# lbarseghyan/diffusion-models

Measured on AMD Instinct MI355X. Metric: sampled images/sec, 32x32 U-Net (dim 64, mults 1-2-4-8), DDPM-1000, higher is better.
Workload: dtype f32; 1 GPU; ddpm1000_32x32_unet64_b256_per_gpu; sampler=p_sample_loop (DDPM), sampler_steps=1000, batch_per_gpu=256, global_batch=256, hip_graph=True, graph_captures=1, parallelism=batch-shard x1, one all-gather per sample()

## Files before the change

### diffusion-models_amd/_lib.py

```python
from __future__ import annotations

import ctypes as C
import os
from typing import Optional

import torch

_HERE = os.path.dirname(os.path.abspath(__file__))
LIB_PATH = os.environ.get("DM_LIB") or os.path.join(_HERE, "libdm_hip.so")
DM_MAX_STAGES = 8
DM_COEFS = 8
DM_EDM_COEFS = 16
EDM_HEUN, EDM_DPMPP = 0, 1
DM_CT_COEFS = 16
CT_PRED_NOISE, CT_PRED_V = 0, 1
DM_REPAINT_COEFS = 16
DM_LV_COEFS = 16
DM_LV_TRAIN_COEFS = 12
DM_WO_COEFS = 16
DM_WO_TRAIN_COEFS = 12
DM_CG_COEFS = 16
ABI_VERSION = 9
DDIM_NO_CLAMP, DDIM_RAW_NOISE = 1, 2

# ... 19 lines not shown
    "dm_op_mse_loss", "dm_op_adam_step", "dm_op_ema_lerp",
    "dm_unet_optimizer_step", "dm_unet_train_scalar", "dm_unet_ema_update", "dm_unet_get_param", "dm_unet_set_train_tensor", "dm_unet_adam_step",
    "dm_unet_train_sync", "dm_unet_check_device_pack",
    "dm_unet_train_dropout", "dm_op_dropout_mask",
    "dm_op_conv2d_bwd", "dm_op_downsample_bwd", "dm_op_block_bwd", "dm_op_rmsnorm_bwd", "dm_op_linear_attention_bwd",
    "dm_op_attention_bwd", "dm_op_cross_attention", "dm_op_cross_attention_bwd",
    "dm_op_linear_attention_core_bwd", "dm_op_attention_core_bwd",
    "dm_profile_enable", "dm_profile_read",
    "dm_unet_forward_ft", "dm_sample_edm",
    "dm_op_edm_churn_in", "dm_op_edm_euler", "dm_op_edm_heun", "dm_op_edm_dpmpp", "dm_op_edm_finalize",
    "dm_unet_train_enable_ft", "dm_unet_loss_backward_edm",
    "dm_op_edm_noise_in", "dm_op_edm_loss", "dm_op_sinusoid_ft_bwd",
    "dm_sample_ct", "dm_unet_loss_backward_ct", "dm_op_ct_step", "dm_op_ct_noise_in", "dm_op_ct_loss",
    "dm_unet_loss_backward_ct_ig", "dm_op_conv7_dgrad", "dm_op_sinusoid_ft_tgrad", "dm_op_ct_sched_reduce",
    "dm_sample_ct_dpmpp", "dm_op_ct_dpmpp_step",
    "dm_unet_optimizer_step_ex",
    "dm_sample_repaint", "dm_op_repaint_step",
    "dm_sample_lv", "dm_unet_loss_backward_lv", "dm_op_lv_step", "dm_op_lv_loss",
    "dm_sample_wo", "dm_unet_loss_backward_wo", "dm_op_wo_step", "dm_op_wo_loss",
    "dm_sample_classifier_guided", "dm_op_cg_mean", "dm_op_cg_finish",
    "dm_op_dpmpp_update",
    "dm_sample_ex_dyn", "dm_op_dyn_threshold", "dm_op_sampler_update_dyn", "dm_op_dpmpp_update_dyn",
    "dm_unet_cond_forward", "dm_unet_cond_backward", "dm_op_deferred_reduce",
)


class UnetCfg(C.Structure):
    _fields_ = [
        ("dim", C.c_int32), ("init_dim", C.c_int32), ("out_dim", C.c_int32), ("channels", C.c_int32),
        ("input_channels", C.c_int32), ("n_stages", C.c_int32),
        ("dim_mults", C.c_int32 * DM_MAX_STAGES), ("full_attn", C.c_int32 * DM_MAX_STAGES),
        ("attn_heads", C.c_int32), ("attn_dim_head", C.c_int32),
        ("text_mode", C.c_int32), ("text_emb_dim", C.c_int32), ("sinusoidal_theta", C.c_float),
        ("learned_sinusoidal_dim", C.c_int32), ("attn_heads_stage", C.c_int32 * DM_MAX_STAGES),
        ("seq1d", C.c_int32),
    ]


class DecoderCfg(C.Structure):
    _fields_ = [
        ("ch", C.c_int32), ("out_ch", C.c_int32), ("n_levels", C.c_int32), ("ch_mult", C.c_int32 * DM_MAX_STAGES),
        ("num_res_blocks", C.c_int32), ("n_attn_res", C.c_int32), ("attn_resolutions", C.c_int32 * DM_MAX_STAGES),
        ("resolution", C.c_int32), ("z_channels", C.c_int32), ("embed_dim", C.c_int32),
    ]


# ... 193 lines not shown
    lib.dm_decoder_create.argtypes = [C.POINTER(DecoderCfg), i32, C.POINTER(vp)]
    lib.dm_decoder_destroy.argtypes = [vp]
    lib.dm_decoder_destroy.restype = None
    lib.dm_decoder_set_param.argtypes = [vp, C.c_char_p, fp, C.POINTER(i64), i32]
    lib.dm_decoder_missing_params.argtypes = [vp]
    lib.dm_decoder_finalize.argtypes = [vp]
    lib.dm_decoder_forward.argtypes = [vp, fp, fp, i32, i32, i32, vp]
    lib.dm_encoder_create.argtypes = [C.POINTER(EncoderCfg), i32, C.POINTER(vp)]
    lib.dm_encoder_destroy.argtypes = [vp]
    lib.dm_encoder_destroy.restype = None
    lib.dm_encoder_set_param.argtypes = [vp, C.c_char_p, fp, C.POINTER(i64), i32]
    lib.dm_encoder_missing_params.argtypes = [vp]
    lib.dm_encoder_finalize.argtypes = [vp]
    lib.dm_encoder_forward.argtypes = [vp, fp, fp, fp, vp, i32, i32, i32, vp]
    lib.dm_encoder_forward_kl.argtypes = [vp, fp, fp, fp, fp, fp, u64, u64, u64, i32, i32, i32, i32, vp]
    lib.dm_encoder_quantize.argtypes = [vp, fp, fp, vp, i32, i32, i32, vp]
    lib.dm_encoder_embed_code.argtypes = [vp, vp, fp, i32, i32, i32, vp]
    lib.dm_op_conv2d.argtypes = [fp, i32, fp, i32, fp, fp, fp, fp, i32, i32, i32, i32, i32, i32, i32, vp]
    lib.dm_op_downsample.argtypes = [fp, i32, fp, fp, fp, i32, i32, i32, i32, vp]
    lib.dm_op_rmsnorm.argtypes = [fp, fp, fp, i32, i32, i32, i32, vp]
    lib.dm_op_block.argtypes = [fp, i32, fp, fp, fp, fp, fp, fp, i32, i32, i32, i32, vp]
    lib.dm_op_linear_attention.argtypes = [fp, fp, fp, fp, fp, fp, fp, fp, i32, i32, i32, i32, i32, i32, vp]
    lib.dm_op_attention.argtypes = [fp, fp, fp, fp, fp, fp, fp, i32, i32, i32, i32, i32, i32, vp]
    lib.dm_op_sampler_update.argtypes = [i32, i32, fp, fp, fp, C.POINTER(C.c_float), fp, fp, i64, vp]
    lib.dm_op_sampler_update_ex.argtypes = [i32, i32, i32, fp, fp, fp, C.POINTER(C.c_float), fp, fp, i64, vp]
    lib.dm_op_conv1d.argtypes = [fp, i32, fp, i32, fp, fp, fp, fp, i32, i32, i32, i32, i32, i32, i32, vp]
    lib.dm_op_block1d.argtypes = [fp, i32, fp, i32, fp, fp, fp, fp, fp, fp, fp, i32, i32, i32, vp]
    lib.dm_op_dpmpp_update.argtypes = [i32, fp, fp, fp, C.POINTER(C.c_float), fp, i64, vp]
    lib.dm_op_dyn_threshold.argtypes = [i32, fp, fp, C.POINTER(C.c_float), i32, i64, C.c_double, fp, vp]
    lib.dm_op_sampler_update_dyn.argtypes = [i32, i32, fp, fp, fp, C.POINTER(C.c_float), fp, i32, i64, fp, fp, vp]
    lib.dm_op_dpmpp_update_dyn.argtypes = [i32, fp, fp, fp, C.POINTER(C.c_float), fp, i32, i64, fp, vp]
    lib.dm_op_cfg_combine.argtypes = [fp, fp, fp, i32, i64, C.c_float, C.c_float, i32, C.c_float, vp]
    lib.dm_op_group_norm.argtypes = [fp, fp, fp, fp, i32, i32, i32, i32, C.c_float, i32, vp]
    lib.dm_op_vae_attention.argtypes = [fp, fp, fp, fp, i32, i32, i32, i32, vp]
    lib.dm_op_vq_nearest.argtypes = [fp, fp, fp, vp, i64, i32, i32, i32, vp]
    lib.dm_op_vq_nearest_nchw.argtypes = [fp, fp, fp, vp, i64, i32, i32, i32, vp]
    lib.dm_op_kl_posterior.argtypes = [fp, i32, fp, u64, u64, u64, i32, fp, fp, fp, i32, i32, i32, vp]
    lib.dm_op_embed_code.argtypes = [vp, i32, fp, fp, i64, i32, i32, i32, vp]
    lib.dm_conv_create.argtypes = [fp, fp, i32, i32, i32, i32, i32, i32, i32, i32, i32, C.POINTER(vp)]
    lib.dm_conv_destroy.argtypes = [vp]
    lib.dm_conv_destroy.restype = None
    lib.dm_conv_forward.argtypes = [vp, fp, i32, i32, i32, i32, fp, vp]
    lib.dm_op_pool2d.argtypes = [fp, fp, i32, i32, i32, i32, i32, i32, i32, i32, vp]
    lib.dm_op_resize_bilinear.argtypes = [fp, fp, i32, i32, i32, i32, i32, i32, fp, fp, vp]
    lib.dm_op_copy_channels_nhwc.argtypes = [fp, i32, fp, i32, i32, i64, vp]
    lib.dm_op_global_avgpool.argtypes = [fp, fp, i32, i32, i32, vp]
# ... 161 lines not shown
```

### diffusion-models_amd/csrc/attn16_fused.hip

```cpp
#include "conv_device.h"

#include <cmath>
#include <cstdlib>
#include <vector>

namespace dm {

static constexpr int A16_OS = 132;
static constexpr int A16_D = 4;

bool attn16_eligible(int dim, int heads, int dh) {
    static const bool off = env_flag("DM_NO_ATTN16");
    return !off && heads == 4 && dh == 32 && dim % 256 == 0 && dim >= 256 && dim <= 1024;
}

void attn16_pack(const float* w_qkv, const float* norm_g, const float* w_out, int C, std::vector<float>& wp,
                 std::vector<float>& wo) {
    const float sc = std::sqrt((float)C), qs = 1.0f / std::sqrt(32.0f);
    wp.assign((size_t)384 * C, 0.f);
    for (int s = 0; s < C / 16; ++s)
        for (int t = 0; t < 24; ++t)
            for (int lane = 0; lane < 64; ++lane)
                for (int j = 0; j < 4; ++j) {
                    const int row = 16 * t + (lane & 15), ch = 16 * s + 4 * (lane >> 4) + j;
                    float v = w_qkv[(size_t)row * C + ch] * norm_g[ch] * sc;
                    if (row < 128) v *= qs;
                    wp[(((size_t)s * 24 + t) * 64 + lane) * 4 + j] = v;
                }
    wo.assign((size_t)C * 128, 0.f);
    for (int s = 0; s < 8; ++s)
        for (int ct = 0; ct < C / 16; ++ct)
            for (int lane = 0; lane < 64; ++lane)
                for (int j = 0; j < 4; ++j)
                    wo[(((size_t)s * (C / 16) + ct) * 64 + lane) * 4 + j] =
                        w_out[(size_t)(16 * ct + (lane & 15)) * 128 + 16 * s + 4 * (lane >> 4) + j];
}

__device__ __forceinline__ f32x4 a16_mfma(float a, float b, f32x4 c) {
    return __builtin_amdgcn_mfma_f32_16x16x4f32(a, b, c, 0, 0, 0);
}

__global__ __launch_bounds__(256) void attn16_fused_kernel(const float* __restrict__ x, const Attn16 w,
                                                            float* __restrict__ y, int add_x) {
    extern __shared__ __attribute__((aligned(16))) float smem[];
    const int C = w.C;
    const int XS = C + 4;
    float* xs = smem;
    float* ol = smem + 16 * XS;
    const int tid = threadIdx.x;
    const int lane = tid & 63;
    const int h = __builtin_amdgcn_readfirstlane(tid >> 6);
    const int l15 = lane & 15, kq = lane >> 4;
    const size_t img = blockIdx.x;

    const int S = C / 16;
    const float* wl = w.wp + (size_t)lane * 4;
    f32x4 wr[A16_D][6];
    auto load = [&](int s, int d) {
        const float* ws = wl + (size_t)s * (24 * 256);
#pragma unroll
        for (int part = 0; part < 3; ++part)
#pragma unroll
            for (int t = 0; t < 2; ++t)
                wr[d][2 * part + t] = *reinterpret_cast<const f32x4*>(ws + (8 * part + 2 * h + t) * 256);
    };
#pragma unroll
    for (int d = 0; d < A16_D; ++d) load(min(d, S - 1), d);

    {
        const int token = tid >> 4, li = tid & 15;
        const float* xr = x + (img * 16 + token) * C;
        f32x4 xv[16];
        float ss = 0.f;
#pragma unroll
        for (int i = 0; i < 16; ++i) {
            const int c = 4 * li + 64 * i;
            if (c < C) {
                xv[i] = *reinterpret_cast<const f32x4*>(xr + c);
                ss += xv[i].x * xv[i].x + xv[i].y * xv[i].y + xv[i].z * xv[i].z + xv[i].w * xv[i].w;
            }
        }
        ss += dpp_f<0xB1>(ss);
        ss += dpp_f<0x4E>(ss);
        ss += dpp_f<0x141>(ss);
        ss += dpp_f<0x140>(ss);
        const float rn = fast_rsq(fmaxf(ss, 1e-24f));
#pragma unroll
        for (int i = 0; i < 16; ++i) {
            const int c = 4 * li + 64 * i;
            if (c < C) *reinterpret_cast<f32x4*>(xs + token * XS + c) = xv[i] * rn;
        }
    }
    __syncthreads();

    const f32x4 z4 = make_f32x4(0.f, 0.f, 0.f, 0.f);
    f32x4 qT[2] = {z4, z4}, kT[2] = {z4, z4}, vv[2] = {z4, z4};
    {
        const float* xrow = xs + l15 * XS + 4 * kq;
        for (int s = 0; s < S; s += A16_D) {
#pragma unroll
            for (int d = 0; d < A16_D; ++d) {
                if (s + d < S) {
                    const f32x4 xa = *reinterpret_cast<const f32x4*>(xrow + 16 * (s + d));
#pragma unroll
                    for (int j = 0; j < 4; ++j) {
#pragma unroll
                        for (int t = 0; t < 2; ++t) {
                            qT[t] = a16_mfma(wr[d][t][j], xa[j], qT[t]);
                            kT[t] = a16_mfma(wr[d][2 + t][j], xa[j], kT[t]);
                            vv[t] = a16_mfma(xa[j], wr[d][4 + t][j], vv[t]);
                        }
                    }
                    if (s + d + A16_D < S) load(s + d + A16_D, d);
                }
            }
        }
    }

    const int CT = C / 16;
    const int ct_per_wave = CT / 4;
    const int n_it = (ct_per_wave / 4) * 8;
    const float* wol = w.wo + (size_t)lane * 4;
    f32x4 wv4[4][4];
    auto load_o = [&](int it, int slot) {
        const int c0 = (it >> 3) * 4, so = it & 7;
#pragma unroll
        for (int i = 0; i < 4; ++i)
            wv4[slot][i] = *reinterpret_cast<const f32x4*>(wol + ((size_t)so * CT + h * ct_per_wave + c0 + i) * 256);
    };
#pragma unroll
    for (int d = 0; d < 4; ++d) load_o(d, d);

    const float* mk = w.mem_kv + (size_t)h * 4 * 32;
    const float* mv = w.mem_kv + (size_t)(4 + h) * 4 * 32;
    f32x4 st = z4, sm = z4;
#pragma unroll
    for (int t = 0; t < 2; ++t) {
        const f32x4 km = l15 < 4 ? *reinterpret_cast<const f32x4*>(mk + l15 * 32 + 16 * t + 4 * kq) : z4;
#pragma unroll
        for (int e = 0; e < 4; ++e) {
            st = a16_mfma(kT[t][e], qT[t][e], st);
            sm = a16_mfma(km[e], qT[t][e], sm);
        }
    }
    const bool g0 = kq == 0;
    float mx = fmaxf(fmaxf(st.x, st.y), fmaxf(st.z, st.w));
    if (g0) mx = fmaxf(mx, fmaxf(fmaxf(sm.x, sm.y), fmaxf(sm.z, sm.w)));
    mx = fmaxf(mx, __shfl_xor(mx, 16));
    mx = fmaxf(mx, __shfl_xor(mx, 32));
    f32x4 pt, pm;
    pt.x = __expf(st.x - mx);
    pt.y = __expf(st.y - mx);
    pt.z = __expf(st.z - mx);
    pt.w = __expf(st.w - mx);
    pm.x = g0 ? __expf(sm.x - mx) : 0.f;
    pm.y = g0 ? __expf(sm.y - mx) : 0.f;
    pm.z = g0 ? __expf(sm.z - mx) : 0.f;
    pm.w = g0 ? __expf(sm.w - mx) : 0.f;
    float sum = (pt.x + pt.y) + (pt.z + pt.w) + (pm.x + pm.y) + (pm.z + pm.w);
    sum += __shfl_xor(sum, 16);
    sum += __shfl_xor(sum, 32);
    const float inv = 1.0f / sum;
    pt = pt * inv;
    pm = pm * inv;

#pragma unroll
    for (int t = 0; t < 2; ++t) {
        f32x4 ot = z4;
        f32x4 vm = z4;
        if (g0) {
            vm.x = mv[0 * 32 + 16 * t + l15];
            vm.y = mv[1 * 32 + 16 * t + l15];
            vm.z = mv[2 * 32 + 16 * t + l15];
            vm.w = mv[3 * 32 + 16 * t + l15];
        }
#pragma unroll
        for (int e = 0; e < 4; ++e) {
            ot = a16_mfma(vv[t][e], pt[e], ot);
            ot = a16_mfma(vm[e], pm[e], ot);
        }
        *reinterpret_cast<f32x4*>(ol + l15 * A16_OS + h * 32 + 16 * t + 4 * kq) = ot;
    }
    __syncthreads();

    f32x4 ob[8];
#pragma unroll
    for (int s = 0; s < 8; ++s) ob[s] = *reinterpret_cast<const f32x4*>(ol + l15 * A16_OS + 16 * s + 4 * kq);
    const size_t row = (img * 16 + l15) * C;
    for (int c0 = 0; c0 < ct_per_wave; c0 += 4) {
        f32x4 acc[4] = {z4, z4, z4, z4};
        const int it0 = (c0 >> 2) * 8;
#pragma unroll
        for (int s = 0; s < 8; ++s) {
#pragma unroll
            for (int j = 0; j < 4; ++j)
#pragma unroll
                for (int i = 0; i < 4; ++i) acc[i] = a16_mfma(wv4[s & 3][i][j], ob[s][j], acc[i]);
            if (it0 + s + 4 < n_it) load_o(it0 + s + 4, s & 3);
        }
#pragma unroll
        for (int i = 0; i < 4; ++i) {
            const int c = 16 * (h * ct_per_wave + c0 + i) + 4 * kq;
            f32x4 r = acc[i] + *reinterpret_cast<const f32x4*>(w.bias + c);
            if (add_x) r += *reinterpret_cast<const f32x4*>(x + row + c);
            *reinterpret_cast<f32x4*>(y + row + c) = r;
        }
    }
}

int launch_attn16_fused(const Attn16& w, const float* x, float* y, int B, bool add_x, hipStream_t s) {
    DM_REQUIRE(w.C % 256 == 0 && w.C >= 256 && w.C <= 1024 && B > 0, "attn16: channel count");
    const size_t lds = (size_t)(16 * (w.C + 4) + 16 * A16_OS) * sizeof(float);
    static LdsOptIn lds_flag;
    if (lds_opt_in(lds_flag, reinterpret_cast<const void*>(attn16_fused_kernel), 1)) return 1;
    const bool timed = prof::enabled();
    if (timed) {
        const double tok = 16.0 * B;
        const double flops = 2.0 * tok * (384.0 * w.C + 128.0 * w.C + 2.0 * 4 * 20 * 32);
        const double bytes = 4.0 * (2.0 * tok * w.C + 512.0 * w.C);
        if (prof::begin("attn16_fused_kernel", flops, bytes, s)) return 1;
    }
    hipLaunchKernelGGL(attn16_fused_kernel, dim3(B), dim3(256), lds, s, x, w, y, add_x ? 1 : 0);
    DM_CHECK_HIP(hipGetLastError());
    if (timed && prof::end(s)) return 1;
    return 0;
}

}
```

### diffusion-models_amd/csrc/dm_api.hip

```cpp
#include "../../include/dm_hip.h"
#include "dm_common.h"
#include "edm.h"
#include "ct.h"
#include "repaint.h"
#include "learned.h"
#include "weighted.h"
#include "cguide.h"

#include <array>
#include <cmath>
#include <cstdlib>
#include <cstring>
#include <functional>
#include <map>
#include <memory>
#include <set>
#include <stdexcept>
#include <string>
#include <unordered_map>
#include <vector>

namespace dm {

static thread_local std::string g_err;
// ... 615 lines not shown
        ob += mb.data.size();
    }
    return 0;
}

static int fuse_linattn(DeviceOwner& own, AttnLayer& A, const float* w_qkv, const float* norm_g, const float* w_out,
                        const float* mem_kv, const float* out_g, int dim, int heads, int dh) {
    A.has_fused = false;
    if (!linattn_fused_eligible(dim, heads, dh)) return 0;
    std::vector<float> wq, wk, wv, wo, kb;
    if (!linattn_fused_pack(w_qkv, norm_g, w_out, mem_kv, dim, wq, wk, wv, wo, kb)) return 0;
    std::vector<float> ogs(out_g, out_g + dim);
    for (float& v : ogs) v *= std::sqrt((float)dim);
    float *dq, *dk, *dv, *dwo, *dkb, *dog;
    if (own.upload(wq.data(), wq.size(), &dq) || own.upload(wk.data(), wk.size(), &dk) ||
        own.upload(wv.data(), wv.size(), &dv) || own.upload(w_out, (size_t)dim * heads * dh, &dwo) ||
        own.upload(kb.data(), kb.size(), &dkb) || own.upload(ogs.data(), ogs.size(), &dog))
        return 1;
    A.fused = LinAttnFused{dim, dq, dk, dv, dwo, A.out.bias, dog, dkb, A.mem_kv};
    A.has_fused = true;
    return 0;
}

static int build_attn_body(dm_unet* u, AttnLayer& A, const std::string& p, int dim, bool full, int heads) {
    A.prefix = p;
    A.full = full;
    A.dim = dim;
    A.heads = heads;
    int hidden = heads * u->dh;
    if (up1(u, p + ".norm.g", &A.norm_g) || up1(u, p + ".mem_kv", &A.mem_kv)) return 1;
    const std::string out = attn_out_param(p, full);
    if (make_conv(u, A.qkv, p + ".to_qkv.weight", "", 3 * hidden, dim, 0, 1, 1, 1, 0, false)) return 1;
    if (make_conv(u, A.out, out + ".weight", out + ".bias", dim, hidden, 0, 1, 1, 1, 0, false)) return 1;
    if (full) {
        A.has16 = false;
        if (attn16_eligible(dim, heads, u->dh)) {
            std::vector<float> wp, wo;
            attn16_pack(P(u, p + ".to_qkv.weight").data.data(), P(u, p + ".norm.g").data.data(),
                        P(u, out + ".weight").data.data(), dim, wp, wo);
            float *dwp, *dwo;
            if (u->own.upload(wp.data(), wp.size(), &dwp) || u->own.upload(wo.data(), wo.size(), &dwo)) return 1;
            A.a16 = Attn16{dim, dwp, dwo, A.out.bias, A.mem_kv};
            A.has16 = true;
        }
    } else {
        if (up1(u, p + ".to_out.1.g", &A.out_g)) return 1;
        if (fuse_linattn(u->own, A, P(u, p + ".to_qkv.weight").data.data(), P(u, p + ".norm.g").data.data(),
                         P(u, out + ".weight").data.data(), P(u, p + ".mem_kv").data.data(),
                         P(u, p + ".to_out.1.g").data.data(), dim, heads, u->dh))
            return 1;
    }
    return 0;
}

static int build_attn1d(dm_unet* u, AttnLayer& A, const std::string& p, int dim, bool full, int heads, int dh) {
    return weight_group(u, p, [&]() -> int {
        const std::string body = p + ".fn.fn", out = attn_out_param(body, full);
        A.prefix = p;
        A.full = full;
        A.dim = dim;
        A.heads = heads;
        A.dh = dh;
        A.mem_kv = nullptr;
        A.has_fused = A.has16 = false;
        if (up1(u, p + ".fn.norm.g", &A.norm_g)) return 1;
        if (make_conv_k(u, A.qkv, body + ".to_qkv.weight", "", 3 * heads * dh, dim, 0, 1, 1, 0)) return 1;
        if (make_conv_k(u, A.out, out + ".weight", out + ".bias", dim, heads * dh, 0, 1, 1, 0)) return 1;
// ... 349 lines not shown
    if (run_conv(c, R.res, x0, x1, H, W, o, EPI_RESIDUAL, nullptr, nullptr, h2)) return 1;
    c.A->release(h2);
    *out = o;
    return 0;
}

static int attn_qkv(Ctx& c, const AttnLayer& At, const float* x, int H, int W, float* xn, float* qkv) {
    const int n = H * W;
    if (!c.dry() && launch_norm_act(x, 1, 0, nullptr, At.norm_g, nullptr, 0, n, nullptr, xn, (int64_t)c.B * n, At.dim, EPI_NORM, c.s))
        return 1;
    return run_conv(c, At.qkv, xn, nullptr, H, W, qkv, 0, nullptr, nullptr, nullptr);
}
static int attn_dh(const dm_unet* u, const AttnLayer& At) { return At.dh ? At.dh : u->dh; }
static int attn_core(Ctx& c, const AttnLayer& At, const float* qkv, int n, float* o, float* ctxws, float* kst) {
    if (c.dry()) return 0;
    const int heads = At.heads, dh = attn_dh(c.u, At), hidden = heads * dh;
    if (!At.full) return launch_linear_attention_core(qkv, At.mem_kv, ctxws, o, c.B, n, heads, dh, c.s, kst);
    const float* mk = At.mem_kv;
    const float* mv = At.mem_kv ? At.mem_kv + (size_t)heads * 4 * dh : nullptr;
    return launch_attention_core(qkv, 3 * hidden, qkv + hidden, qkv + 2 * hidden, 3 * hidden, mk, mv, At.mem_kv ? 4 : 0, o, hidden,
                                 c.B, n, n, heads, dh, 1.0f / sqrtf((float)dh), c.s);
}

static int run_attn(Ctx& c, const AttnLayer& At, const float* x, int H, int W, float** out, bool add_x = true) {
    const int res_flag = add_x ? EPI_RESIDUAL : 0;
    const float* xres = add_x ? x : nullptr;
    dm_unet* u = c.u;
    const int n = H * W, heads = At.heads, dh = attn_dh(u, At), hidden = heads * dh;
    const size_t rows = (size_t)c.B * n;
    if (!At.full && At.has_fused) {
        float* ws = c.A->alloc(linattn_fused_ws_floats(c.B, n));
        float* yf = c.A->alloc(rows * At.dim);
        if (!c.dry() && launch_linattn_fused(At.fused, x, ws, yf, c.B, n, add_x, c.s)) return 1;
        c.A->release(ws);
        *out = yf;
        return 0;
    }
    if (At.full && At.has16 && n == 16) {
        float* yf = c.A->alloc(rows * At.dim);
        if (!c.dry() && launch_attn16_fused(At.a16, x, yf, c.B, add_x, c.s)) return 1;
        *out = yf;
        return 0;
    }
    float* xn = c.A->alloc(rows * At.dim);
    float* qkv = c.A->alloc(rows * 3 * hidden);
    float* o = c.A->alloc(rows * hidden);
    float* y = c.A->alloc(rows * At.dim);
    if (attn_qkv(c, At, x, H, W, xn, qkv)) return 1;
    if (At.full) {
        if (attn_core(c, At, qkv, n, o, nullptr, nullptr)) return 1;
        if (run_conv(c, At.out, o, nullptr, H, W, y, res_flag, nullptr, nullptr, xres)) return 1;
    } else {
        float* ctxws = c.A->alloc((size_t)c.B * heads * dh * dh);
        if (attn_core(c, At, qkv, n, o, ctxws, nullptr)) return 1;
        if (run_conv(c, At.out, o, nullptr, H, W, y, EPI_NORM | res_flag, At.out_g, nullptr, xres)) return 1;
        c.A->release(ctxws);
    }
    c.A->release(xn);
    c.A->release(qkv);
    c.A->release(o);
    *out = y;
    return 0;
}
// ... 496 lines not shown
```

### diffusion-models_amd/csrc/dm_common.h

```cpp
#pragma once

#include <hip/hip_runtime.h>
#include <stdint.h>

#include <string>
#include <vector>

#include <cstdlib>

namespace dm {

inline int env_int(const char* name, int dflt) {
    const char* e = std::getenv(name);
    return e ? std::atoi(e) : dflt;
}
inline bool env_flag(const char* name) { return std::getenv(name) != nullptr; }

__device__ __forceinline__ float relu_f(float v) { return v < 0.0f ? 0.0f : v; }

void set_error(const std::string& msg);

#define DM_CHECK_HIP(expr)                                                                  \
    do {                                                                                    \
        hipError_t _e = (expr);                                                             \
// ... 108 lines not shown

bool init7_eligible(int Cout, int C0, int C1, int KH, int KW, int stride, int pad, bool up);
size_t init7_packed_floats(int Cin);
void init7_pack_weights(const float* oihw, float* packed, int Cin);
int init7_launch(const ConvParams& p, hipStream_t s);
int launch_conv7_dgrad(const float* dy_nhwc, const float* w_oihw, float* dx_nchw, int B, int H, int W, int Cout, int C,
                       hipStream_t s);

bool pw_eligible(int Cout, int C0, int C1, int KH, int KW, int stride, int pad, bool up);
size_t pw_packed_floats(int Cout, int C0, int C1);
void pw_pack_weights(const float* oihw, float* packed, int Cout, int C0, int C1);
bool pw_s2d_eligible(int Cout, int C0, int C1, int KH, int KW, int stride, int pad, bool up);
void pw_pack_weights_s2d(const float* oihw, float* packed, int Cout, int C0);
ConvGeom pw_plan(int B, int Ho, int Wo, int Cout, int C0, int C1, bool allow_split);
bool pw_shape_ok(int B, int Ho, int Wo, int Cout, int C0, int C1);
int pw_launch(const ConvParams& p, hipStream_t s);

struct Attn16 {
    int C;
    const float* wp;
    const float* wo;
    const float* bias;
    const float* mem_kv;
};
bool attn16_eligible(int dim, int heads, int dh);
void attn16_pack(const float* w_qkv, const float* norm_g, const float* w_out, int C, std::vector<float>& wp,
                 std::vector<float>& wo);
int launch_attn16_fused(const Attn16& w, const float* x, float* y, int B, bool add_x, hipStream_t s);

bool upwino_eligible(int Cout, int C0, int C1, int KH, int KW, int stride, int pad, bool up);
size_t upwino_packed_floats(int Cout, int C0, int C1);
void upwino_pack_weights(const float* oihw, float* packed, int Cout, int C0, int C1);
ConvGeom upwino_plan(int B, int Hl, int Wl, int Cout, int C0, int C1, bool allow_split);
bool upwino_shape_ok(int B, int Hl, int Wl, int Cout, int C0, int C1);
int upwino_launch(const ConvParams& p, hipStream_t s);

namespace prof {
bool enabled();
bool detail();
int begin(const char* kernel, double flops, double bytes, hipStream_t s);
int end(hipStream_t s);
}

int launch_nchw_to_nhwc(const float* in, float* out, int B, int C, int HW, hipStream_t s);
int launch_nhwc_to_nchw(const float* in, float* out, int B, int C, int HW, hipStream_t s);
int launch_norm_act(const float* x, int nsplit, int64_t split_stride, const float* bias, const float* g,
                    const float* scale, int ss_stride, int pix_per_image, const float* residual, float* y,
                    int64_t rows, int C, int flags, hipStream_t s, int res_nsplit = 1, int64_t res_stride = 0,
                    const float* res_bias = nullptr);
int launch_linear_rows(const float* x, int ldx, const float* W, const float* bias, float* y, int ldy, int R, int I,
                       int O, int act_in, int act_out, hipStream_t s);
// ... 240 lines not shown
```

### diffusion-models_amd/csrc/dm_ops.inc

```
namespace dm {

static int d2h(const float* dev, size_t n, std::vector<float>& out) {
    out.resize(n);
    if (n) DM_CHECK_HIP(hipMemcpy(out.data(), dev, n * sizeof(float), hipMemcpyDeviceToHost));
    return 0;
}

template <class F>
static int run_op(hipStream_t s, F body) {
    Arena dry;
    dry.dry = true;
    if (body(dry)) return 1;
    void* buf = nullptr;
    DM_CHECK_HIP(hipMalloc(&buf, dry.off + 256));
    Arena A;
    A.base = static_cast<char*>(buf);
    A.cap = dry.off + 256;
    hipError_t e = hipMemsetAsync(buf, 0xFF, A.cap, s);
    int rc = 0;
    if (e == hipSuccess) {
        rc = body(A);
        e = hipStreamSynchronize(s);
    }
    (void)hipFree(buf);
// ... 161 lines not shown
        Ctx c{&dummy, &A, s, B, nullptr, 0};
        float* a = to_nhwc(A, x, B, C, H * W, s, &rc);
        if (rc) return 1;
        float* y = nullptr;
        if (run_attn(c, At, a, H, W, &y, false)) return 1;
        if (!A.dry && launch_nhwc_to_nchw(y, out, B, C, H * W, s)) return 1;
        return 0;
    });
}

int dm_op_linear_attention(const float* x, const float* norm_g, const float* mem_kv, const float* w_qkv,
                           const float* w_out, const float* b_out, const float* out_g, float* out, int B, int C,
                           int H, int W, int heads, int dim_head, void* stream) {
    DM_REQUIRE(out_g, "null argument");
    return attn_op(false, x, norm_g, mem_kv, w_qkv, w_out, b_out, out_g, out, B, C, H, W, heads, dim_head, stream);
}

int dm_op_attention(const float* x, const float* norm_g, const float* mem_kv, const float* w_qkv,
                    const float* w_out, const float* b_out, float* out, int B, int C, int H, int W, int heads,
                    int dim_head, void* stream) {
    return attn_op(true, x, norm_g, mem_kv, w_qkv, w_out, b_out, nullptr, out, B, C, H, W, heads, dim_head, stream);
}

int dm_profile_enable(int on) {
    prof::g_on = on != 0;
    prof::g_detail = on == 2;
    if (on) {
        constexpr int N = 33;
        hipEvent_t e0[N], e1[N];
        for (int i = 0; i < N; ++i) {
            DM_CHECK_HIP(hipEventCreate(&e0[i]));
            DM_CHECK_HIP(hipEventCreate(&e1[i]));
        }
        if (launch_spin(2.0, nullptr)) return 1;
        for (int i = 0; i < N; ++i) {
            DM_CHECK_HIP(hipEventRecord(e0[i], nullptr));
            if (launch_spin(0.0, nullptr)) return 1;
            DM_CHECK_HIP(hipEventRecord(e1[i], nullptr));
        }
        DM_CHECK_HIP(hipDeviceSynchronize());
        std::vector<float> ms(N);
        for (int i = 0; i < N; ++i) {
            DM_CHECK_HIP(hipEventElapsedTime(&ms[i], e0[i], e1[i]));
            (void)hipEventDestroy(e0[i]);
            (void)hipEventDestroy(e1[i]);
        }
// ... 198 lines not shown
```

### include/dm_hip.h

```cpp
#ifndef DM_HIP_H
#define DM_HIP_H

#include <stdint.h>

#ifdef __cplusplus
extern "C" {
#endif

#define DM_MAX_STAGES 8

#define DM_TEXT_NONE 0
#define DM_TEXT_CONCAT 1
#define DM_TEXT_CROSS 2

typedef struct dm_unet_cfg {
    int32_t dim;
    int32_t init_dim;
    int32_t out_dim;
    int32_t channels;
    int32_t input_channels;
    int32_t n_stages;
    int32_t dim_mults[DM_MAX_STAGES];
    int32_t full_attn[DM_MAX_STAGES];
    int32_t attn_heads;
// ... 133 lines not shown
int dm_encoder_finalize(dm_encoder* e);
int dm_encoder_forward(dm_encoder* e, const float* x, float* zq, float* pre_quant, int32_t* indices, int B, int H, int W,
                       void* stream);
int dm_encoder_forward_kl(dm_encoder* e, const float* x, float* moments_nchw, float* z, float* kl, const float* eps,
                          uint64_t seed, uint64_t draw, uint64_t element_offset, int sample, int B, int H, int W, void* stream);
int dm_encoder_quantize(dm_encoder* e, const float* h_nchw, float* zq, int32_t* indices, int B, int h, int w, void* stream);
int dm_encoder_embed_code(dm_encoder* e, const int64_t* indices, float* out, int B, int h, int w, void* stream);


int dm_op_conv2d(const float* in0, int C0, const float* in1, int C1, const float* weight, const float* bias,
                 const float* residual, float* out, int B, int H, int W, int Cout, int ksize, int pad, int up2,
                 void* stream);
int dm_op_downsample(const float* in, int C, const float* weight, const float* bias, float* out, int B, int H,
                     int W, int Cout, void* stream);
int dm_op_rmsnorm(const float* x, const float* g, float* out, int B, int C, int H, int W, void* stream);
int dm_op_block(const float* x, int Cin, const float* weight, const float* bias, const float* g,
                const float* scale, const float* shift, float* out, int B, int H, int W, int Cout, void* stream);
int dm_op_linear_attention(const float* x, const float* norm_g, const float* mem_kv, const float* w_qkv,
                           const float* w_out, const float* b_out, const float* out_g, float* out, int B, int C,
                           int H, int W, int heads, int dim_head, void* stream);
int dm_op_attention(const float* x, const float* norm_g, const float* mem_kv, const float* w_qkv,
                    const float* w_out, const float* b_out, float* out, int B, int C, int H, int W, int heads,
                    int dim_head, void* stream);
int dm_op_sampler_update(int kind, int objective, const float* x, const float* eps, const float* noise,
                         const float* c_host, float* out, float* x_start, int64_t n, void* stream);
int dm_op_sampler_update_ex(int kind, int objective, int ddim_flags, const float* x, const float* eps, const float* noise,
                            const float* c_host, float* out, float* x_start, int64_t n, void* stream);
int dm_op_conv1d(const float* in0, int C0, const float* in1, int C1, const float* weight, const float* bias,
                 const float* residual, float* out, int B, int L, int Cout, int K, int stride, int pad, int up2,
                 void* stream);
int dm_op_block1d(const float* x0, int C0, const float* x1, int C1, const float* weight, const float* bias, const float* g,
                  const float* scale, const float* shift, const float* residual, float* out, int B, int L, int Cout,
                  void* stream);
int dm_op_dpmpp_update(int objective, const float* x, const float* model_out, float* x0_hist, const float* coef_host,
                       float* out, int64_t n, void* stream);
int dm_op_dyn_threshold(int objective, const float* x, const float* model_out, const float* c_host, int B, int64_t per,
                        double percentile, float* s_out, void* stream);
int dm_op_sampler_update_dyn(int kind, int objective, const float* x, const float* eps, const float* noise,
                             const float* c_host, const float* s, int B, int64_t per, float* out, float* x_start,
                             void* stream);
int dm_op_dpmpp_update_dyn(int objective, const float* x, const float* model_out, float* x0_hist, const float* coef_host,
                           const float* s, int B, int64_t per, float* out, void* stream);
int dm_op_cfg_combine(const float* cond, const float* null_out, float* out, int B, int64_t per_sample, float cond_scale,
                      float rescaled_phi, int remove_parallel_component, float keep_parallel_frac, void* stream);
int dm_op_group_norm(const float* x_nhwc, const float* weight, const float* bias, float* y_nhwc, int B, int HW, int C,
                     int groups, float eps, int swish, void* stream);
// ... 451 lines not shown
```

Measured before the change: 58.75 images/s.

## Split 16-token attention across heads with grouped images and separate out-projection

Adds a heads-split form of the 16-token full-attention kernel. Each block handles one head for G images, and the four waves split the input-channel reduction for QKV and combine partial sums through LDS. The output projection then runs as a separate pointwise conv with a residual epilogue, and this path is used for dims 256/512 when batch is at least 32. The aim is more parallelism and reuse of each head's weights across images, at the cost of an extra kernel launch and an intermediate buffer round-trip to memory.

```diff
diff --git a/diffusion-models_amd/_lib.py b/diffusion-models_amd/_lib.py
--- a/diffusion-models_amd/_lib.py
+++ b/diffusion-models_amd/_lib.py
@@ -65,6 +65,7 @@
     "dm_op_dpmpp_update",
     "dm_sample_ex_dyn", "dm_op_dyn_threshold", "dm_op_sampler_update_dyn", "dm_op_dpmpp_update_dyn",
     "dm_unet_cond_forward", "dm_unet_cond_backward", "dm_op_deferred_reduce",
+    "dm_op_attention16",
 )
 
 
@@ -304,6 +305,8 @@
     lib.dm_op_block.argtypes = [fp, i32, fp, fp, fp, fp, fp, fp, i32, i32, i32, i32, vp]
     lib.dm_op_linear_attention.argtypes = [fp, fp, fp, fp, fp, fp, fp, fp, i32, i32, i32, i32, i32, i32, vp]
     lib.dm_op_attention.argtypes = [fp, fp, fp, fp, fp, fp, fp, i32, i32, i32, i32, i32, i32, vp]
+    if hasattr(lib, "dm_op_attention16"):
+        lib.dm_op_attention16.argtypes = [fp, fp, fp, fp, fp, fp, fp, i32, i32, i32, i32, vp]
     lib.dm_op_sampler_update.argtypes = [i32, i32, fp, fp, fp, C.POINTER(C.c_float), fp, fp, i64, vp]
     lib.dm_op_sampler_update_ex.argtypes = [i32, i32, i32, fp, fp, fp, C.POINTER(C.c_float), fp, fp, i64, vp]
     lib.dm_op_conv1d.argtypes = [fp, i32, fp, i32, fp, fp, fp, fp, i32, i32, i32, i32, i32, i32, i32, vp]
diff --git a/diffusion-models_amd/csrc/attn16_fused.hip b/diffusion-models_amd/csrc/attn16_fused.hip
--- a/diffusion-models_amd/csrc/attn16_fused.hip
+++ b/diffusion-models_amd/csrc/attn16_fused.hip
@@ -40,99 +40,12 @@
     return __builtin_amdgcn_mfma_f32_16x16x4f32(a, b, c, 0, 0, 0);
 }
 
-__global__ __launch_bounds__(256) void attn16_fused_kernel(const float* __restrict__ x, const Attn16 w,
-                                                            float* __restrict__ y, int add_x) {
-    extern __shared__ __attribute__((aligned(16))) float smem[];
-    const int C = w.C;
-    const int XS = C + 4;
-    float* xs = smem;
-    float* ol = smem + 16 * XS;
-    const int tid = threadIdx.x;
-    const int lane = tid & 63;
-    const int h = __builtin_amdgcn_readfirstlane(tid >> 6);
+__device__ __forceinline__ void a16_softmax_o(const f32x4 (&qT)[2], const f32x4 (&kT)[2], const f32x4 (&vv)[2],
+                                              const float* __restrict__ mem_kv, int h, int lane, f32x4 (&ot)[2]) {
     const int l15 = lane & 15, kq = lane >> 4;
-    const size_t img = blockIdx.x;
-
-    const int S = C / 16;
-    const float* wl = w.wp + (size_t)lane * 4;
-    f32x4 wr[A16_D][6];
-    auto load = [&](int s, int d) {
-        const float* ws = wl + (size_t)s * (24 * 256);
-#pragma unroll
-        for (int part = 0; part < 3; ++part)
-#pragma unroll
-            for (int t = 0; t < 2; ++t)
-                wr[d][2 * part + t] = *reinterpret_cast<const f32x4*>(ws + (8 * part + 2 * h + t) * 256);
-    };
-#pragma unroll
-    for (int d = 0; d < A16_D; ++d) load(min(d, S - 1), d);
-
-    {
-        const int token = tid >> 4, li = tid & 15;
-        const float* xr = x + (img * 16 + token) * C;
-        f32x4 xv[16];
-        float ss = 0.f;
-#pragma unroll
-        for (int i = 0; i < 16; ++i) {
-            const int c = 4 * li + 64 * i;
-            if (c < C) {
-                xv[i] = *reinterpret_cast<const f32x4*>(xr + c);
-                ss += xv[i].x * xv[i].x + xv[i].y * xv[i].y + xv[i].z * xv[i].z + xv[i].w * xv[i].w;
-            }
-        }
-        ss += dpp_f<0xB1>(ss);
-        ss += dpp_f<0x4E>(ss);
-        ss += dpp_f<0x141>(ss);
-        ss += dpp_f<0x140>(ss);
-        const float rn = fast_rsq(fmaxf(ss, 1e-24f));
-#pragma unroll
-        for (int i = 0; i < 16; ++i) {
-            const int c = 4 * li + 64 * i;
-            if (c < C) *reinterpret_cast<f32x4*>(xs + token * XS + c) = xv[i] * rn;
-        }
-    }
-    __syncthreads();
-
     const f32x4 z4 = make_f32x4(0.f, 0.f, 0.f, 0.f);
-    f32x4 qT[2] = {z4, z4}, kT[2] = {z4, z4}, vv[2] = {z4, z4};
-    {
-        const float* xrow = xs + l15 * XS + 4 * kq;
-        for (int s = 0; s < S; s += A16_D) {
-#pragma unroll
-            for (int d = 0; d < A16_D; ++d) {
-                if (s + d < S) {
-                    const f32x4 xa = *reinterpret_cast<const f32x4*>(xrow + 16 * (s + d));
-#pragma unroll
-                    for (int j = 0; j < 4; ++j) {
-#pragma unroll
-                        for (int t = 0; t < 2; ++t) {
-                            qT[t] = a16_mfma(wr[d][t][j], xa[j], qT[t]);
-                            kT[t] = a16_mfma(wr[d][2 + t][j], xa[j], kT[t]);
-                            vv[t] = a16_mfma(xa[j], wr[d][4 + t][j], vv[t]);
-                        }
-                    }
-                    if (s + d + A16_D < S) load(s + d + A16_D, d);
-                }
-            }
-        }
-    }
-
-    const int CT = C / 16;
-    const int ct_per_wave = CT / 4;
-    const int n_it = (ct_per_wave / 4) * 8;
-    const float* wol = w.wo + (size_t)lane * 4;
-    f32x4 wv4[4][4];
-    auto load_o = [&](int it, int slot) {
-        const int c0 = (it >> 3) * 4, so = it & 7;
-#pragma unroll
-        for (int i = 0; i < 4; ++i)
-            wv4[slot][i] = *reinterpret_cast<const f32x4*>(wol + ((size_t)so * CT + h * ct_per_wave + c0 + i) * 256);
-    };
-#pragma unroll
-    for (int d = 0; d < 4; ++d) load_o(d, d);
-
-    const float* mk = w.mem_kv + (size_t)h * 4 * 32;
-    const float* mv = w.mem_kv + (size_t)(4 + h) * 4 * 32;
+    const float* mk = mem_kv + (size_t)h * 4 * 32;
+    const float* mv = mem_kv + (size_t)(4 + h) * 4 * 32;
     f32x4 st = z4, sm = z4;
 #pragma unroll
     for (int t = 0; t < 2; ++t) {
@@ -166,7 +79,7 @@
 
 #pragma unroll
     for (int t = 0; t < 2; ++t) {
-        f32x4 ot = z4;
+        ot[t] = z4;
         f32x4 vm = z4;
         if (g0) {
             vm.x = mv[0 * 32 + 16 * t + l15];
@@ -176,11 +89,107 @@
         }
 #pragma unroll
         for (int e = 0; e < 4; ++e) {
-            ot = a16_mfma(vv[t][e], pt[e], ot);
-            ot = a16_mfma(vm[e], pm[e], ot);
-        }
-        *reinterpret_cast<f32x4*>(ol + l15 * A16_OS + h * 32 + 16 * t + 4 * kq) = ot;
-    }
+            ot[t] = a16_mfma(vv[t][e], pt[e], ot[t]);
+            ot[t] = a16_mfma(vm[e], pm[e], ot[t]);
+        }
+    }
+}
+
+__global__ __launch_bounds__(256) void attn16_fused_kernel(const float* __restrict__ x, const Attn16 w,
+                                                            float* __restrict__ y, int add_x) {
+    extern __shared__ __attribute__((aligned(16))) float smem[];
+    const int C = w.C;
+    const int XS = C + 4;
+    float* xs = smem;
+    float* ol = smem + 16 * XS;
+    const int tid = threadIdx.x;
+    const int lane = tid & 63;
+    const int h = __builtin_amdgcn_readfirstlane(tid >> 6);
+    const int l15 = lane & 15, kq = lane >> 4;
+    const size_t img = blockIdx.x;
+
+    const int S = C / 16;
+    const float* wl = w.wp + (size_t)lane * 4;
+    f32x4 wr[A16_D][6];
+    auto load = [&](int s, int d) {
+        const float* ws = wl + (size_t)s * (24 * 256);
+#pragma unroll
+        for (int part = 0; part < 3; ++part)
+#pragma unroll
+            for (int t = 0; t < 2; ++t)
+                wr[d][2 * part + t] = *reinterpret_cast<const f32x4*>(ws + (8 * part + 2 * h + t) * 256);
+    };
+#pragma unroll
+    for (int d = 0; d < A16_D; ++d) load(min(d, S - 1), d);
+
+    {
+        const int token = tid >> 4, li = tid & 15;
+        const float* xr = x + (img * 16 + token) * C;
+        f32x4 xv[16];
+        float ss = 0.f;
+#pragma unroll
+        for (int i = 0; i < 16; ++i) {
+            const int c = 4 * li + 64 * i;
+            if (c < C) {
+                xv[i] = *reinterpret_cast<const f32x4*>(xr + c);
+                ss += xv[i].x * xv[i].x + xv[i].y * xv[i].y + xv[i].z * xv[i].z + xv[i].w * xv[i].w;
+            }
+        }
+        ss += dpp_f<0xB1>(ss);
+        ss += dpp_f<0x4E>(ss);
+        ss += dpp_f<0x141>(ss);
+        ss += dpp_f<0x140>(ss);
+        const float rn = fast_rsq(fmaxf(ss, 1e-24f));
+#pragma unroll
+        for (int i = 0; i < 16; ++i) {
+            const int c = 4 * li + 64 * i;
+            if (c < C) *reinterpret_cast<f32x4*>(xs + token * XS + c) = xv[i] * rn;
+        }
+    }
+    __syncthreads();
+
+    const f32x4 z4 = make_f32x4(0.f, 0.f, 0.f, 0.f);
+    f32x4 qT[2] = {z4, z4}, kT[2] = {z4, z4}, vv[2] = {z4, z4};
+    {
+        const float* xrow = xs + l15 * XS + 4 * kq;
+        for (int s = 0; s < S; s += A16_D) {
+#pragma unroll
+            for (int d = 0; d < A16_D; ++d) {
+                if (s + d < S) {
+                    const f32x4 xa = *reinterpret_cast<const f32x4*>(xrow + 16 * (s + d));
+#pragma unroll
+                    for (int j = 0; j < 4; ++j) {
+#pragma unroll
+                        for (int t = 0; t < 2; ++t) {
+                            qT[t] = a16_mfma(wr[d][t][j], xa[j], qT[t]);
+                            kT[t] = a16_mfma(wr[d][2 + t][j], xa[j], kT[t]);
+                            vv[t] = a16_mfma(xa[j], wr[d][4 + t][j], vv[t]);
+                        }
+                    }
+                    if (s + d + A16_D < S) load(s + d + A16_D, d);
+                }
+            }
+        }
+    }
+
+    const int CT = C / 16;
+    const int ct_per_wave = CT / 4;
+    const int n_it = (ct_per_wave / 4) * 8;
+    const float* wol = w.wo + (size_t)lane * 4;
+    f32x4 wv4[4][4];
+    auto load_o = [&](int it, int slot) {
+        const int c0 = (it >> 3) * 4, so = it & 7;
+#pragma unroll
+        for (int i = 0; i < 4; ++i)
+            wv4[slot][i] = *reinterpret_cast<const f32x4*>(wol + ((size_t)so * CT + h * ct_per_wave + c0 + i) * 256);
+    };
+#pragma unroll
+    for (int d = 0; d < 4; ++d) load_o(d, d);
+
+    f32x4 ot[2];
+    a16_softmax_o(qT, kT, vv, w.mem_kv, h, lane, ot);
+#pragma unroll
+    for (int t = 0; t < 2; ++t) *reinterpret_cast<f32x4*>(ol + l15 * A16_OS + h * 32 + 16 * t + 4 * kq) = ot[t];
     __syncthreads();
 
     f32x4 ob[8];
@@ -226,4 +235,169 @@
     return 0;
 }
 
-}
+bool attn16_heads_eligible(int dim) { return dim == 256 || dim == 512; }
+
+void attn16_pack_heads(const float* w_qkv, const float* norm_g, int C, std::vector<float>& wph) {
+    const float sc = std::sqrt((float)C), qs = 1.0f / std::sqrt(32.0f);
+    const int S = C / 16;
+    wph.assign((size_t)384 * C, 0.f);
+    for (int h = 0; h < 4; ++h)
+        for (int s = 0; s < S; ++s)
+            for (int t = 0; t < 6; ++t)
+                for (int lane = 0; lane < 64; ++lane)
+                    for (int j = 0; j < 4; ++j) {
+                        const int row = 128 * (t / 2) + 32 * h + 16 * (t % 2) + (lane & 15), ch = 16 * s + 4 * (lane >> 4) + j;
+                        float v = w_qkv[(size_t)row * C + ch] * norm_g[ch] * sc;
+                        if (row < 128) v *= qs;
+                        wph[((((size_t)h * S + s) * 6 + t) * 64 + lane) * 4 + j] = v;
+                    }
+}
+
+static size_t a16_heads_lds_floats(int C, int G) {
+    const size_t xs = (size_t)16 * G * (C + 4), parts = (size_t)4 * G * 6 * 256;
+    return xs > parts ? xs : parts;
+}
+
+template <int G>
+__global__ __launch_bounds__(256) void attn16_heads_kernel(const float* __restrict__ x, const Attn16 w, float* __restrict__ o,
+                                                            int B) {
+    extern __shared__ __attribute__((aligned(16))) float smem[];
+    const int C = w.C;
+    const int XS = C + 4;
+    const int tid = threadIdx.x;
+    const int lane = tid & 63;
+    const int wave = __builtin_amdgcn_readfirstlane(tid >> 6);
+    const int l15 = lane & 15, kq = lane >> 4;
+    const int h = blockIdx.x & 3;
+    const int img0 = (blockIdx.x >> 2) * G;
+    const int nreal = min(G, B - img0);
+
+    const int S = C / 16, SW = S / 4;
+    const float* wl = w.wph + ((size_t)h * S + (size_t)wave * SW) * (6 * 256) + (size_t)lane * 4;
+    f32x4 wr[A16_D][6];
+    auto load = [&](int i, int d) {
+#pragma unroll
+        for (int t = 0; t < 6; ++t) wr[d][t] = *reinterpret_cast<const f32x4*>(wl + ((size_t)i * 6 + t) * 256);
+    };
+#pragma unroll
+    for (int d = 0; d < A16_D; ++d) load(d, d);
+
+    {
+        const int token = tid >> 4, li = tid & 15;
+        f32x4 xg[G][8];
+#pragma unroll
+        for (int g = 0; g < G; ++g) {
+            if (g < nreal) {
+                const float* xr = x + ((size_t)(img0 + g) * 16 + token) * C;
+#pragma unroll
+                for (int i = 0; i < 8; ++i) {
+                    const int c = 4 * li + 64 * i;
+                    if (c < C) xg[g][i] = *reinterpret_cast<const f32x4*>(xr + c);
+                }
+            }
+        }
+#pragma unroll
+        for (int g = 0; g < G; ++g) {
+            if (g < nreal) {
+                f32x4(&xv)[8] = xg[g];
+                float ss = 0.f;
+#pragma unroll
+                for (int i = 0; i < 8; ++i) {
+                    const int c = 4 * li + 64 * i;
+                    if (c < C) ss += xv[i].x * xv[i].x + xv[i].y * xv[i].y + xv[i].z * xv[i].z + xv[i].w * xv[i].w;
+                }
+                ss += dpp_f<0xB1>(ss);
+                ss += dpp_f<0x4E>(ss);
+                ss += dpp_f<0x141>(ss);
+                ss += dpp_f<0x140>(ss);
+                const float rn = fast_rsq(fmaxf(ss, 1e-24f));
+#pragma unroll
+                for (int i = 0; i < 8; ++i) {
+                    const int c = 4 * li + 64 * i;
+                    if (c < C) *reinterpret_cast<f32x4*>(smem + (g * 16 + token) * XS + c) = xv[i] * rn;
+                }
+            }
+        }
+    }
+    __syncthreads();
+
+    const f32x4 z4 = make_f32x4(0.f, 0.f, 0.f, 0.f);
+    f32x4 acc[G][6];
+#pragma unroll
+    for (int g = 0; g < G; ++g)
+#pragma unroll
+        for (int t = 0; t < 6; ++t) acc[g][t] = z4;
+    {
+        const float* xrow = smem + l15 * XS + 4 * kq + 16 * wave * SW;
+        for (int i0 = 0; i0 < SW; i0 += A16_D) {
+#pragma unroll
+            for (int d = 0; d < A16_D; ++d) {
+                const int i = i0 + d;
+                f32x4 xa[G];
+#pragma unroll
+                for (int g = 0; g < G; ++g)
+                    if (g < nreal) xa[g] = *reinterpret_cast<const f32x4*>(xrow + g * 16 * XS + 16 * i);
+#pragma unroll
+                for (int g = 0; g < G; ++g) {
+                    if (g < nreal) {
+#pragma unroll
+                        for (int j = 0; j < 4; ++j) {
+#pragma unroll
+                            for (int t = 0; t < 4; ++t) acc[g][t] = a16_mfma(wr[d][t][j], xa[g][j], acc[g][t]);
+#pragma unroll
+                            for (int t = 4; t < 6; ++t) acc[g][t] = a16_mfma(xa[g][j], wr[d][t][j], acc[g][t]);
+                        }
+                    }
+                }
+                if (i + A16_D < SW) load(i + A16_D, d);
+            }
+        }
+    }
+
+    __syncthreads();
+#pragma unroll
+    for (int g = 0; g < G; ++g)
+        if (g < nreal)
+#pragma unroll
+            for (int t = 0; t < 6; ++t) *reinterpret_cast<f32x4*>(smem + (((wave * G + g) * 6 + t) * 64 + lane) * 4) = acc[g][t];
+    __syncthreads();
+    if (wave >= nreal) return;
+
+    f32x4 pr[6];
+#pragma unroll
+    for (int t = 0; t < 6; ++t) {
+        auto part = [&](int ws) { return *reinterpret_cast<const f32x4*>(smem + (((ws * G + wave) * 6 + t) * 64 + lane) * 4); };
+        pr[t] = ((part(0) + part(1)) + part(2)) + part(3);
+    }
+    const f32x4 qT[2] = {pr[0], pr[1]}, kT[2] = {pr[2], pr[3]}, vv[2] = {pr[4], pr[5]};
+    f32x4 ot[2];
+    a16_softmax_o(qT, kT, vv, w.mem_kv, h, lane, ot);
+    float* orow = o + ((size_t)(img0 + wave) * 16 + l15) * 128 + h * 32 + 4 * kq;
+#pragma unroll
+    for (int t = 0; t < 2; ++t) *reinterpret_cast<f32x4*>(orow + 16 * t) = ot[t];
+}
+
+int launch_attn16_heads(const Attn16& w, const float* x, float* o, int B, int G, hipStream_t s) {
+    DM_REQUIRE(attn16_heads_eligible(w.C) && w.wph && B > 0 && (G == 2 || G == 4), "attn16 heads form: shape");
+    const size_t lds = a16_heads_lds_floats(w.C, G) * sizeof(float);
+    static LdsOptIn lds_flag;
+    if (lds_opt_in(lds_flag, reinterpret_cast<const void*>(attn16_heads_kernel<2>), 1)) return 1;
+    if (lds_opt_in(lds_flag, reinterpret_cast<const void*>(attn16_heads_kernel<4>), 2)) return 1;
+    const bool timed = prof::enabled();
+    if (timed) {
+        const double tok = 16.0 * B;
+        const double flops = 2.0 * tok * (384.0 * w.C + 2.0 * 4 * 20 * 32);
+        const double bytes = 4.0 * (tok * (w.C + 128.0) + 384.0 * w.C);
+        if (prof::begin(G == 4 ? "attn16_heads_kernel<4>" : "attn16_heads_kernel<2>", flops, bytes, s)) return 1;
+    }
+    const dim3 grid(4 * ((B + G - 1) / G));
+    if (G == 4)
+        hipLaunchKernelGGL(attn16_heads_kernel<4>, grid, dim3(256), lds, s, x, w, o, B);
+    else
+        hipLaunchKernelGGL(attn16_heads_kernel<2>, grid, dim3(256), lds, s, x, w, o, B);
+    DM_CHECK_HIP(hipGetLastError());
+    if (timed && prof::end(s)) return 1;
+    return 0;
+}
+
+}
diff --git a/diffusion-models_amd/csrc/dm_api.hip b/diffusion-models_amd/csrc/dm_api.hip
--- a/diffusion-models_amd/csrc/dm_api.hip
+++ b/diffusion-models_amd/csrc/dm_api.hip
@@ -661,6 +661,23 @@
     return 0;
 }
 
+static int fuse_attn16(DeviceOwner& own, AttnLayer& A, const float* w_qkv, const float* norm_g, const float* w_out, int dim,
+                       int heads, int dh) {
+    A.has16 = false;
+    if (!A.mem_kv || !attn16_eligible(dim, heads, dh)) return 0;
+    std::vector<float> wp, wo, wph;
+    attn16_pack(w_qkv, norm_g, w_out, dim, wp, wo);
+    float *dwp, *dwo, *dwph = nullptr;
+    if (own.upload(wp.data(), wp.size(), &dwp) || own.upload(wo.data(), wo.size(), &dwo)) return 1;
+    if (attn16_heads_eligible(dim) && A.out.packed[CONV_PW]) {
+        attn16_pack_heads(w_qkv, norm_g, dim, wph);
+        if (own.upload(wph.data(), wph.size(), &dwph)) return 1;
+    }
+    A.a16 = Attn16{dim, dwp, dwo, A.out.bias, A.mem_kv, dwph};
+    A.has16 = true;
+    return 0;
+}
+
 static int build_attn_body(dm_unet* u, AttnLayer& A, const std::string& p, int dim, bool full, int heads) {
     A.prefix = p;
     A.full = full;
@@ -672,16 +689,9 @@
     if (make_conv(u, A.qkv, p + ".to_qkv.weight", "", 3 * hidden, dim, 0, 1, 1, 1, 0, false)) return 1;
     if (make_conv(u, A.out, out + ".weight", out + ".bias", dim, hidden, 0, 1, 1, 1, 0, false)) return 1;
     if (full) {
-        A.has16 = false;
-        if (attn16_eligible(dim, heads, u->dh)) {
-            std::vector<float> wp, wo;
-            attn16_pack(P(u, p + ".to_qkv.weight").data.data(), P(u, p + ".norm.g").data.data(),
-                        P(u, out + ".weight").data.data(), dim, wp, wo);
-            float *dwp, *dwo;
-            if (u->own.upload(wp.data(), wp.size(), &dwp) || u->own.upload(wo.data(), wo.size(), &dwo)) return 1;
-            A.a16 = Attn16{dim, dwp, dwo, A.out.bias, A.mem_kv};
-            A.has16 = true;
-        }
+        if (fuse_attn16(u->own, A, P(u, p + ".to_qkv.weight").data.data(), P(u, p + ".norm.g").data.data(),
+                        P(u, out + ".weight").data.data(), dim, heads, u->dh))
+            return 1;
     } else {
         if (up1(u, p + ".to_out.1.g", &A.out_g)) return 1;
         if (fuse_linattn(u->own, A, P(u, p + ".to_qkv.weight").data.data(), P(u, p + ".norm.g").data.data(),
@@ -1077,7 +1087,13 @@
                                  c.B, n, n, heads, dh, 1.0f / sqrtf((float)dh), c.s);
 }
 
-static int run_attn(Ctx& c, const AttnLayer& At, const float* x, int H, int W, float** out, bool add_x = true) {
+static int a16_heads_form(int B, int C) {
+    (void)C;
+    return B >= 32 ? 2 : 0;
+}
+
+static int run_attn(Ctx& c, const AttnLayer& At, const float* x, int H, int W, float** out, bool add_x = true,
+                    int a16_form = -1) {
     const int res_flag = add_x ? EPI_RESIDUAL : 0;
     const float* xres = add_x ? x : nullptr;
     dm_unet* u = c.u;
@@ -1092,8 +1108,16 @@
         return 0;
     }
     if (At.full && At.has16 && n == 16) {
+        const int G = !At.a16.wph ? 0 : a16_form >= 0 ? a16_form : a16_heads_form(c.B, At.dim);
         float* yf = c.A->alloc(rows * At.dim);
-        if (!c.dry() && launch_attn16_fused(At.a16, x, yf, c.B, add_x, c.s)) return 1;
+        if (G) {
+            float* o = c.A->alloc(rows * hidden);
+            if (!c.dry() && launch_attn16_heads(At.a16, x, o, c.B, G, c.s)) return 1;
+            if (run_conv(c, At.out, o, nullptr, H, W, yf, res_flag, nullptr, nullptr, xres)) return 1;
+            c.A->release(o);
+        } else if (!c.dry() && launch_attn16_fused(At.a16, x, yf, c.B, add_x, c.s)) {
+            return 1;
+        }
         *out = yf;
         return 0;
     }
diff --git a/diffusion-models_amd/csrc/dm_common.h b/diffusion-models_amd/csrc/dm_common.h
--- a/diffusion-models_amd/csrc/dm_common.h
+++ b/diffusion-models_amd/csrc/dm_common.h
@@ -154,11 +154,15 @@
     const float* wo;
     const float* bias;
     const float* mem_kv;
+    const float* wph;
 };
 bool attn16_eligible(int dim, int heads, int dh);
 void attn16_pack(const float* w_qkv, const float* norm_g, const float* w_out, int C, std::vector<float>& wp,
                  std::vector<float>& wo);
 int launch_attn16_fused(const Attn16& w, const float* x, float* y, int B, bool add_x, hipStream_t s);
+bool attn16_heads_eligible(int dim);
+void attn16_pack_heads(const float* w_qkv, const float* norm_g, int C, std::vector<float>& wph);
+int launch_attn16_heads(const Attn16& w, const float* x, float* o, int B, int G, hipStream_t s);
 
 bool upwino_eligible(int Cout, int C0, int C1, int KH, int KW, int stride, int pad, bool up);
 size_t upwino_packed_floats(int Cout, int C0, int C1);
diff --git a/diffusion-models_amd/csrc/dm_ops.inc b/diffusion-models_amd/csrc/dm_ops.inc
--- a/diffusion-models_amd/csrc/dm_ops.inc
+++ b/diffusion-models_amd/csrc/dm_ops.inc
@@ -207,6 +207,39 @@
     return attn_op(true, x, norm_g, mem_kv, w_qkv, w_out, b_out, nullptr, out, B, C, H, W, heads, dim_head, stream);
 }
 
+int dm_op_attention16(const float* x, const float* norm_g, const float* mem_kv, const float* w_qkv, const float* w_out,
+                      const float* b_out, float* out, int B, int C, int add_x, int form, void* stream) {
+    DM_REQUIRE(x && norm_g && mem_kv && w_qkv && w_out && b_out && out && B > 0, "null argument");
+    DM_REQUIRE(form == -1 || form == 0 || form == 2 || form == 4, "form: -1, 0, 2 or 4");
+    DM_REQUIRE(attn16_eligible(C, 4, 32), "attention16: C must be 256, 512, 768 or 1024");
+    DM_REQUIRE(form <= 0 || attn16_heads_eligible(C), "attention16: the heads form takes C = 256 or 512");
+    hipStream_t s = static_cast<hipStream_t>(stream);
+    std::vector<float> wq, wo, bo, ng;
+    if (d2h(w_qkv, (size_t)384 * C, wq) || d2h(w_out, (size_t)C * 128, wo) || d2h(b_out, C, bo) || d2h(norm_g, C, ng)) return 1;
+    dm_unet dummy;
+    init_dummy(dummy, 4, 32);
+    AttnLayer At;
+    At.full = true;
+    At.dim = C;
+    At.heads = 4;
+    At.norm_g = const_cast<float*>(norm_g);
+    At.mem_kv = const_cast<float*>(mem_kv);
+    if (make_conv(dummy.own, At.qkv, wq.data(), nullptr, 384, C, 0, 1, 1, 1, 0, false)) return 1;
+    if (make_conv(dummy.own, At.out, wo.data(), bo.data(), C, 128, 0, 1, 1, 1, 0, false)) return 1;
+    if (fuse_attn16(dummy.own, At, wq.data(), ng.data(), wo.data(), C, 4, 32)) return 1;
+    DM_REQUIRE(At.has16, "attention16: the layer did not take the 16-token form");
+    return run_op(s, [&](Arena& A) -> int {
+        int rc = 0;
+        Ctx c{&dummy, &A, s, B, nullptr, 0};
+        float* a = to_nhwc(A, x, B, C, 16, s, &rc);
+        if (rc) return 1;
+        float* y = nullptr;
+        if (run_attn(c, At, a, 4, 4, &y, add_x != 0, form)) return 1;
+        if (!A.dry && launch_nhwc_to_nchw(y, out, B, C, 16, s)) return 1;
+        return 0;
+    });
+}
+
 int dm_profile_enable(int on) {
     prof::g_on = on != 0;
     prof::g_detail = on == 2;
diff --git a/include/dm_hip.h b/include/dm_hip.h
--- a/include/dm_hip.h
+++ b/include/dm_hip.h
@@ -179,6 +179,8 @@
 int dm_op_attention(const float* x, const float* norm_g, const float* mem_kv, const float* w_qkv,
                     const float* w_out, const float* b_out, float* out, int B, int C, int H, int W, int heads,
                     int dim_head, void* stream);
+int dm_op_attention16(const float* x, const float* norm_g, const float* mem_kv, const float* w_qkv, const float* w_out,
+                      const float* b_out, float* out, int B, int C, int add_x, int form, void* stream);
 int dm_op_sampler_update(int kind, int objective, const float* x, const float* eps, const float* noise,
                          const float* c_host, float* out, float* x_start, int64_t n, void* stream);
 int dm_op_sampler_update_ex(int kind, int objective, int ddim_flags, const float* x, const float* eps, const float* noise,
```

Result: no change. 58.90 images/s (median of 6 runs) (+0.3%).
